# KTH-RPL/cloth-splatting

Hardware: AMD Instinct MI355X
Metric: rasterizer fwd+bwd rendered Mpix/s (scene_1, 800x800) (higher is better)
Workload: dtype f32

## Files before the change

### cloth-splatting_amd/csrc/csplat_k8_views_body.h

```cpp
    constexpr bool STAGE = true;
    if (tab.valid && *tab.valid == 0u) return;
    const int bx = (int)blockIdx.x + block0;
    const unsigned smask = tab.sharedmask;
    const bool put3 = !UNREAD && tab.unread == 0u;
#define PUTL(local, ptr, idx, val, bit)                                                    \
    do {                                                                                   \
        if (smask & (bit)) (local) += (val);                                               \
        else { float *p_ = (ptr) + (idx); *p_ = (accmask & (bit)) ? *p_ + (val) : (val); } \
    } while (0)
    static_assert(VL == 4 && K8_MAX_VIEWS <= 2 * VL, "one quad per Gaussian, at most two views per lane");
    constexpr int NG = NT / VL;
    __shared__ float s_in[STAGE ? NG * SH_ROW : 1];
    __shared__ float s_cam[CAM ? K8_MAX_VIEWS * NG * CAM_NC : 1];
    __shared__ float s_cpart[CAM ? CAM_PARTS * CAM_NC : 1];
    const int gi = threadIdx.x / VL, vl = threadIdx.x % VL;
    const int i = bx * NG + gi;
    const int rows = min(NG, P - bx * NG);
    if (STAGE) {
        stage_sh_rows<NT>(shs + (size_t)bx * NG * 48, rows, s_in);
        __syncthreads();
    }
    if (i < P) {
    float L_op = 0.f, L_col[3] = {0.f, 0.f, 0.f}, L_m3[3] = {0.f, 0.f, 0.f}, L_c6[6] = {0.f, 0.f, 0.f, 0.f, 0.f, 0.f};
    float L_sc[3] = {0.f, 0.f, 0.f}, L_rt[4] = {0.f, 0.f, 0.f, 0.f};
    bool vis_n = false;
    float a9_n[9];
    float dz_n = 0.f;
    auto load_record = [](const float *acc_, int i_, float (&a)[9], float &dz_) {
        const float4 *r4 = reinterpret_cast<const float4 *>(acc_ + (size_t)i_ * ACC_STRIDE);
        const float4 q0 = r4[0], q1 = r4[1], q2 = r4[2];
        a[0] = q0.x; a[1] = q0.y; a[2] = q0.z; a[3] = q0.w; a[4] = q1.x; a[5] = q1.y; a[6] = q1.z; a[7] = q1.w; a[8] = q2.x;
        if constexpr (DEPTH) dz_ = q2.y;
    };
    float e0[6] = {0.f, 0.f, 0.f, 0.f, 0.f, 0.f};
    if (vl < tab.n) {
        vis_n = tab.v[vl].radii[i] > 0;
        load_record(tab.v[vl].acc, i, a9_n, dz_n);
        if (vis_n && (tab.v[vl].accmask & CSPLAT_SCRATCH_ZEROED)) clear_record(tab.v[vl].acc, i);
    }
    for (int vi = vl; vi < tab.n; vi += VL) {
    const K8View &w = tab.v[vi];
    const Cam cam = w.cam;
    const Geom g = w.g;
    const int32_t *radii = w.radii;
    const float *acc = w.acc, *means3D = w.means3D, *rotations = w.rotations;
    float *dL_dmean2D = w.dL_dmean2D, *dL_dconic = w.dL_dconic, *dL_dopacity = w.dL_dopacity, *dL_dcolor = w.dL_dcolor;
    float *dL_dmean3D = w.dL_dmean3D, *dL_dcov3D = w.dL_dcov3D, *dL_dscale = w.dL_dscale, *dL_drot = w.dL_drot;
    const unsigned accmask = w.accmask;
    (void)radii; (void)acc;
    const bool vis = vis_n;
    float *const crow = s_cam + (CAM ? (vi * NG + gi) * CAM_NC : 0);
    float a9[9];
#pragma unroll
    for (int k = 0; k < 9; k++) a9[k] = vis ? a9_n[k] : 0.f;
    const float dz = vis ? dz_n : 0.f;
    moments_to_gradients(a9, vis ? g.conic_opacity[i] : make_float4(0.f, 0.f, 0.f, 0.f));
    a9[0] *= (float)cam.W; a9[1] *= (float)cam.H;
    if (vi + VL < tab.n) {
        const K8View &wn = tab.v[vi + VL];
        vis_n = wn.radii[i] > 0;
        load_record(wn.acc, i, a9_n, dz_n);
        if (vis_n && (wn.accmask & CSPLAT_SCRATCH_ZEROED)) clear_record(wn.acc, i);
    }
    dL_dmean2D[3 * i] = a9[0]; dL_dmean2D[3 * i + 1] = a9[1]; dL_dmean2D[3 * i + 2] = 0.f;
    if (put3) { dL_dconic[4 * i] = a9[2]; dL_dconic[4 * i + 1] = a9[3]; dL_dconic[4 * i + 2] = 0.f; dL_dconic[4 * i + 3] = a9[4]; }
    if constexpr (!AA) PUTL(L_op, dL_dopacity, i, a9[5], CSPLAT_ACC_OPACITY);
    if (put3) {
        PUTL(L_col[0], dL_dcolor, 3 * i, a9[6], CSPLAT_ACC_COLOR); PUTL(L_col[1], dL_dcolor, 3 * i + 1, a9[7], CSPLAT_ACC_COLOR);
        PUTL(L_col[2], dL_dcolor, 3 * i + 2, a9[8], CSPLAT_ACC_COLOR);
    }

// ... 3 lines not shown
    if (!vis) {
        if constexpr (AA) PUTL(L_op, dL_dopacity, i, 0.f, CSPLAT_ACC_OPACITY);
#pragma unroll
        for (int k = 0; k < 3; k++) PUTL(L_m3[k], dL_dmean3D, 3 * i + k, 0.f, CSPLAT_ACC_MEAN3D);
        if (put3)
#pragma unroll
            for (int k = 0; k < 6; k++) PUTL(L_c6[k], dL_dcov3D, 6 * i + k, 0.f, CSPLAT_ACC_COV3D);
        if (dL_dscale)
#pragma unroll
            for (int k = 0; k < 3; k++) PUTL(L_sc[k], dL_dscale, 3 * i + k, 0.f, CSPLAT_ACC_SCALE);
        if (dL_drot)
#pragma unroll
            for (int k = 0; k < 4; k++) PUTL(L_rt[k], dL_drot, 4 * i + k, 0.f, CSPLAT_ACC_ROT);
        if constexpr (CAM) cam_partials_zero(crow);
    } else {
    const float p[3] = {means3D[3 * i], means3D[3 * i + 1], means3D[3 * i + 2]};
    const float *view = cam.view, *proj = cam.proj;

    {
        float pv[3];
        view_point(p, view, pv);
        ProjJac pj;
        proj_jacobian(pv, cam, pj);
        float c6[6];
#pragma unroll
        for (int k = 0; k < 6; k++) c6[k] = g.cov3D[6 * i + k];
        float a, b, c;
        float aa_ga = 0.f, aa_gb = 0.f, aa_gc = 0.f;
        if constexpr (AA) {
            float a0, c0;
            cov2d_undilated(c6, pj, a0, b, c0);
            a = a0 + AA_DILATE; c = c0 + AA_DILATE;
            const float h = aa_backward(a0, b, c0, aa_opacities[i] * a9[5], aa_ga, aa_gb, aa_gc);
            PUTL(L_op, dL_dopacity, i, h * a9[5], CSPLAT_ACC_OPACITY);
        } else {
            cov2d_from_cov3d(c6, pj, a, b, c);
        }
        const float denom = a * c - b * b;
        const float denom2inv = 1.0f / ((denom * denom) + 0.0000001f);
        const float gcx = a9[2], gcy = a9[3], gcz = a9[4];
        float dL_da = 0.f, dL_db = 0.f, dL_dc = 0.f;
        const float *t0 = pj.t0, *t1 = pj.t1;
        if (denom2inv != 0.f) {
            dL_da = denom2inv * (-c * c * gcx + 2.f * b * c * gcy + (denom - a * c) * gcz);
            dL_dc = denom2inv * (-a * a * gcz + 2.f * a * b * gcy + (denom - a * c) * gcx);
            dL_db = denom2inv * 2.f * (b * c * gcx - (denom + 2.f * b * b) * gcy + a * b * gcz);
            if constexpr (AA) { dL_da += aa_ga; dL_db += aa_gb; dL_dc += aa_gc; }
            g6[0] = t0[0] * t0[0] * dL_da + t0[0] * t1[0] * dL_db + t1[0] * t1[0] * dL_dc;
// ... 30 lines not shown
            cam_partials_view(crow, p, dpv, cam.fx * tz, -(cam.fx * pj.tx) * tz2, cam.fy * tz, -(cam.fy * pj.ty) * tz2, dT0, dT1);
        }
    }
    {
        const float hw = proj[3] * p[0] + proj[7] * p[1] + proj[11] * p[2] + proj[15];
        const float m_w = 1.0f / (hw + 0.0000001f);
        const float mul1 = (proj[0] * p[0] + proj[4] * p[1] + proj[8] * p[2] + proj[12]) * m_w * m_w;
        const float mul2 = (proj[1] * p[0] + proj[5] * p[1] + proj[9] * p[2] + proj[13]) * m_w * m_w;
        const float gx2 = a9[0], gy2 = a9[1];
        dmean[0] += (proj[0] * m_w - proj[3] * mul1) * gx2 + (proj[1] * m_w - proj[3] * mul2) * gy2;
        dmean[1] += (proj[4] * m_w - proj[7] * mul1) * gx2 + (proj[5] * m_w - proj[7] * mul2) * gy2;
        dmean[2] += (proj[8] * m_w - proj[11] * mul1) * gx2 + (proj[9] * m_w - proj[11] * mul2) * gy2;
        if constexpr (CAM) cam_partials_proj(crow, p, gx2 * m_w, gy2 * m_w, -(mul1 * gx2 + mul2 * gy2));
    }
    if constexpr (CAM) { crow[32] = 0.f; crow[33] = 0.f; crow[34] = 0.f; }
    if (shs && dL_dsh) {
        const float *sh = (const float *)(s_in + gi * SH_ROW);
        const uint32_t cl = g.clamped[i];
        const float vx = p[0] - cam.campos[0], vy = p[1] - cam.campos[1], vz = p[2] - cam.campos[2];
        const float sum2 = vx * vx + vy * vy + vz * vz;
        const float len = sqrtf(sum2);
        const float x = vx / len, y = vy / len, z = vz / len;
        float ddx = 0.f, ddy = 0.f, ddz = 0.f;
        e[0] = x; e[1] = y; e[2] = z;
#pragma unroll
        for (int ch = 0; ch < 3; ch++) {
            const float dRGB = ((cl >> ch) & 1u) ? 0.f : a9[6 + ch];
            e[3 + ch] = dRGB;
            float dx_ = 0.f, dy_ = 0.f, dz_ = 0.f;
#define S(k) sh[(k) * 3 + ch]
            if (D > 0) {
                dx_ = -SH_C1 * S(3); dy_ = -SH_C1 * S(1); dz_ = SH_C1 * S(2);
                if (D > 1) {
// ... 22 lines not shown
        dmean[1] += (-vx * vy * ddx + (sum2 - vy * vy) * ddy - vz * vy * ddz) * invsum32;
        dmean[2] += (-vx * vz * ddx - vy * vz * ddy + (sum2 - vz * vz) * ddz) * invsum32;
        if constexpr (CAM) {
            const float dd = x * ddx + y * ddy + z * ddz, il = 1.f / len;
            crow[32] = (x * dd - ddx) * il; crow[33] = (y * dd - ddy) * il; crow[34] = (z * dd - ddz) * il;
        }
    }
    if constexpr (DEPTH) { dmean[0] += dz * view[2]; dmean[1] += dz * view[6]; dmean[2] += dz * view[10]; }
#pragma unroll
    for (int k = 0; k < 3; k++) PUTL(L_m3[k], dL_dmean3D, 3 * i + k, dmean[k], CSPLAT_ACC_MEAN3D);
    if (put3)
#pragma unroll
        for (int k = 0; k < 6; k++) PUTL(L_c6[k], dL_dcov3D, 6 * i + k, g6[k], CSPLAT_ACC_COV3D);

    if (!use_precomp_cov && dL_dscale && dL_drot) {
        const float q[4] = {rotations[4 * i], rotations[4 * i + 1], rotations[4 * i + 2], rotations[4 * i + 3]};
        float R[3][3];
        quat_to_rot(q, R);
        const float s[3] = {scale_mod * scales[3 * i], scale_mod * scales[3 * i + 1], scale_mod * scales[3 * i + 2]};
        const float dS[3][3] = {{g6[0], 0.5f * g6[1], 0.5f * g6[2]},
                                {0.5f * g6[1], g6[3], 0.5f * g6[4]},
                                {0.5f * g6[2], 0.5f * g6[4], g6[5]}};
        float dA[3][3];
#pragma unroll
        for (int r = 0; r < 3; r++)
#pragma unroll
            for (int k = 0; k < 3; k++)
                dA[r][k] = 2.f * (dS[r][0] * R[0][k] * s[k] + dS[r][1] * R[1][k] * s[k] + dS[r][2] * R[2][k] * s[k]);
#pragma unroll
        for (int k = 0; k < 3; k++) PUTL(L_sc[k], dL_dscale, 3 * i + k, dA[0][k] * R[0][k] + dA[1][k] * R[1][k] + dA[2][k] * R[2][k], CSPLAT_ACC_SCALE);
        float dR[3][3];
#pragma unroll
        for (int r = 0; r < 3; r++)
#pragma unroll
// ... 5 lines not shown
        const float dq2 = 2.f * (-2.f * qy * dR[0][0] + qx * dR[0][1] + qr * dR[0][2] + qx * dR[1][0] + qz * dR[1][2] -
                                    qr * dR[2][0] + qz * dR[2][1] - 2.f * qy * dR[2][2]);
        const float dq3 = 2.f * (-2.f * qz * dR[0][0] - qr * dR[0][1] + qx * dR[0][2] + qr * dR[1][0] - 2.f * qz * dR[1][1] +
                                    qy * dR[1][2] + qx * dR[2][0] + qy * dR[2][1]);
        PUTL(L_rt[0], dL_drot, 4 * i, dq0, CSPLAT_ACC_ROT); PUTL(L_rt[1], dL_drot, 4 * i + 1, dq1, CSPLAT_ACC_ROT);
        PUTL(L_rt[2], dL_drot, 4 * i + 2, dq2, CSPLAT_ACC_ROT); PUTL(L_rt[3], dL_drot, 4 * i + 3, dq3, CSPLAT_ACC_ROT);
    }
    }
    if (vi < VL) {
#pragma unroll
        for (int k = 0; k < 6; k++) e0[k] = e[k];
    } else {
#pragma unroll
        for (int k = 0; k < 6; k++) s_in[gi * SH_ROW + vl * 6 + k] = e[k];
    }
    }
    __builtin_amdgcn_wave_barrier();
    if (VL == 4) {
        auto quad_sum = [](float v) {
            v += __int_as_float(__builtin_amdgcn_update_dpp(0, __float_as_int(v), 0xB1, 0xF, 0xF, false));
            v += __int_as_float(__builtin_amdgcn_update_dpp(0, __float_as_int(v), 0x4E, 0xF, 0xF, false));
            return v;
        };
        L_op = quad_sum(L_op);
#pragma unroll
        for (int k = 0; k < 3; k++) { L_col[k] = quad_sum(L_col[k]); L_m3[k] = quad_sum(L_m3[k]); L_sc[k] = quad_sum(L_sc[k]); }
#pragma unroll
        for (int k = 0; k < 6; k++) L_c6[k] = quad_sum(L_c6[k]);
#pragma unroll
        for (int k = 0; k < 4; k++) L_rt[k] = quad_sum(L_rt[k]);
// ... 62 lines not shown
            for (int k = 0; k < 3; k++) PUTS(w.dL_dcolor, 3 * i + k, L_col[k], CSPLAT_ACC_COLOR);
#pragma unroll
        for (int k = 0; k < 3; k++) PUTS(w.dL_dmean3D, 3 * i + k, L_m3[k], CSPLAT_ACC_MEAN3D);
        if (put3)
#pragma unroll
            for (int k = 0; k < 6; k++) PUTS(w.dL_dcov3D, 6 * i + k, L_c6[k], CSPLAT_ACC_COV3D);
        if (w.dL_dscale)
#pragma unroll
            for (int k = 0; k < 3; k++) PUTS(w.dL_dscale, 3 * i + k, L_sc[k], CSPLAT_ACC_SCALE);
        if (w.dL_drot)
#pragma unroll
            for (int k = 0; k < 4; k++) PUTS(w.dL_drot, 4 * i + k, L_rt[k], CSPLAT_ACC_ROT);
#undef PUTS
    }
    }
    if constexpr (CAM)
        for (int vi = 0; vi < tab.n; vi++) cam_block_sum<NT>(s_cam + vi * NG * CAM_NC, rows, s_cpart, cam_slabs->p[vi] + (size_t)bx * CAM_NC);
#undef PUTL
```

### cloth-splatting_amd/csrc/csplat_raster.hip

```cpp
#include "csplat_common.h"

#include <atomic>
#include <cstring>
#include <chrono>
#include <mutex>
#include <type_traits>

#include "csplat_raster_math.h"
#include "csplat_raster_k1.h"
#include "csplat_raster_binning.h"
#include "csplat_raster_k5b_k6.h"

namespace {

constexpr int ACC_STRIDE = 16;

#define CSPLAT_ROWMASK_OP(OP, dst, src0, src1, RM)                                                                                  \
    asm("s_nop 1\n\tv_" OP "_f32_dpp %0, %1, %2 quad_perm:[0,1,2,3] row_mask:" RM " bank_mask:0xf" : "+v"(dst) : "v"(src0), "v"(src1))
__device__ __forceinline__ void rows_scan_mul(float f, float Tin, float &Tr, float &Tout) {
    const auto s16 = __builtin_amdgcn_permlane16_swap(__float_as_uint(f), __float_as_uint(f), false, false);
    const float ev = __uint_as_float(s16[0]), od = __uint_as_float(s16[1]);
    const float pr = ev * od;
    const auto s32 = __builtin_amdgcn_permlane32_swap(__float_as_uint(pr), __float_as_uint(pr), false, false);
    const float lo = __uint_as_float(s32[0]), hi = __uint_as_float(s32[1]);
// ... 597 lines not shown
        g_mail.tried = true;
        void *h = nullptr, *d = nullptr;
        if (hipHostMalloc(&h, MAIL_SLOTS * MAIL_WORDS * 4, hipHostMallocMapped | hipHostMallocPortable) == hipSuccess &&
            hipHostGetDevicePointer(&d, h, 0) == hipSuccess) {
            memset(h, 0, MAIL_SLOTS * MAIL_WORDS * 4);
            g_mail.host = (volatile uint32_t *)h;
            g_mail.dev = (uint32_t *)d;
        }
        (void)hipGetLastError();
    }
    return g_mail.host != nullptr;
}

unsigned long long *g_stamp_buf = nullptr;
size_t g_stamp_words = 0;

int tsort_mode(int P) { return (P < (1 << 24) ? 1 : 0) | (dbg(CSPLAT_DEBUG_SORT_RADIX_ONLY) ? 2 : 0) | (dbg(CSPLAT_DEBUG_SORT_RADIX_FALLBACK) ? 4 : 0); }

int higher_msb(uint32_t n) {
    int b = 0;
    while ((1u << b) < n && b < 31) b++;
    return b == 0 ? 1 : b;
}

hipEvent_t pooled_event() {
    constexpr int N = 256;
    static hipEvent_t ring[N];
    static std::atomic<unsigned> next{0};
    static std::mutex mu;
    const unsigned k = next.fetch_add(1) % N;
// ... 188 lines not shown
    for (int i = 0; i < V; i++) {
        const FwdTicket &t = g_tickets[tk[i]];
        K1View &k = tab.v[i];
        k.means3D = t.means3D; k.rotations = t.rotations; k.cam = t.cam; k.g = t.g; k.radii = t.radii; k.table = t.table;
        k.info = t.info; k.mailbox = t.mb_dev; k.ranges = t.ranges; k.tag = t.tag;
    }
    {
        ProfScope ps(PROF_K1, join);
        const bool stage = a.M == 16 && ((uintptr_t)a.shs & 15u) == 0;
        if (a.aa && stage)
            k_preprocess_views_aa<true><<<cdiv(P, K1V_G), 256, 0, join>>>(P, a.D, a.M, a.shs, a.opacities, a.scales, a.scale_modifier, tab,
                                                                        nocull_mode());
        else if (a.aa)
            k_preprocess_views_aa<false><<<cdiv(P, K1V_G), 256, 0, join>>>(P, a.D, a.M, a.shs, a.opacities, a.scales, a.scale_modifier, tab,
                                                                         nocull_mode());
        else if (stage)
            k_preprocess_views<true><<<cdiv(P, K1V_G), 256, 0, join>>>(P, a.D, a.M, a.shs, a.opacities, a.scales, a.scale_modifier, tab,
                                                                     nocull_mode());
        else
            k_preprocess_views<false><<<cdiv(P, K1V_G), 256, 0, join>>>(P, a.D, a.M, a.shs, a.opacities, a.scales, a.scale_modifier, tab,
                                                                      nocull_mode());
        LAUNCH_CHECK();
    }
    {
        ProfScope ps(PROF_K2, join);
        k_tile_count_views<<<dim3(nb, V), BUCKET_G, (size_t)tiles * 4, join>>>(P, tiles, tab);
        LAUNCH_CHECK();
        k_tile_colscan_views<<<dim3(cdiv(tiles, 256), V), 256, 0, join>>>(tiles, nb, tab);
        LAUNCH_CHECK();
        k_tile_scan_views<<<V, 1024, 0, join>>>(tiles, nb, tab);
// ... 849 lines not shown
    if (b_hi <= b_lo) return 0;
    auto go = [&](auto kernel, auto... extra) {
        kernel<<<b_hi - b_lo, 128, 0, join>>>(a.P, a.D, a.M, a.shs, a.scales, a.scale_modifier, 0, a.dL_dsh, tab, b_lo, extra...);
    };
    if (aa_of(a)) {
        if (depth && cam_k8) go(k_preprocess_bwd_views_aa<128, 4, true, true>, sl, a.opacities);
        else if (depth) go(k_preprocess_bwd_views_aa<128, 4, true, false>, sl, a.opacities);
        else if (cam_k8) go(k_preprocess_bwd_views_aa<128, 4, false, true>, sl, a.opacities);
        else go(k_preprocess_bwd_views_aa<128, 4, false, false>, sl, a.opacities);
    } else if (cam_k8) {
        if (depth) go(k_preprocess_bwd_views_cam<128, 4, true>, sl);
        else go(k_preprocess_bwd_views_cam<128, 4, false>, sl);
    } else if (depth) {
        go(k_preprocess_bwd_views_depth<128, 4>);
    } else {
        if (tab.unread) go(k_preprocess_bwd_views<128, 4, true>);
        else go(k_preprocess_bwd_views<128, 4, false>);
    }
    LAUNCH_CHECK();
    return 0;
}

struct GroupPlan {
    bool want_k7, want_k8, whole, shared, one_k8, det_mode, cam, cam_k8, feat;
    ScratchPath path;
    K8Table tab;
};
static void plan_group(int V, const csplat_view *v, unsigned parts, int nslices, GroupPlan &g) {
    g.want_k7 = (parts & 1u) != 0; g.want_k8 = (parts & 2u) != 0; g.whole = parts == 3u && nslices == 1;
    g.shared = false;
    for (int i = 0; i < V; i++) g.shared |= (v[i].accmask & ~(unsigned)(CSPLAT_SCRATCH_ZEROED | CSPLAT_K8_OUTPUTS_UNREAD)) != 0u;
// ... 287 lines not shown
```

### cloth-splatting_amd/csrc/csplat_raster_k1.h

```cpp
#pragma once

namespace {

template <bool STAGE, bool AA = false>
__device__ __forceinline__ void preprocess_body(int P, int D, int M, const float *__restrict__ means3D,
                                                const float *__restrict__ shs,
                                                const float *__restrict__ colors_precomp,
                                                const float *__restrict__ opacities,
                                                const float *__restrict__ scales, float scale_mod,
                                                const float *__restrict__ rotations,
                                                const float *__restrict__ cov3D_precomp, const Cam &cam, const Geom &g,
                                                int32_t *__restrict__ radii, int nocull, const float *s_shrows, int i, int srow) {
#pragma clang fp contract(off)
    if (i >= P) return;
    float depth = 0.f, px = 0.f, py = 0.f, cut = -1.f;
    float4 co = {0.f, 0.f, 0.f, 0.f};
    float rgb[3] = {0.f, 0.f, 0.f};
    float c6[6] = {0.f, 0.f, 0.f, 0.f, 0.f, 0.f};
    uint32_t clampbits = 0, touched = 0;
    int rad = 0;

    const float p[3] = {means3D[3 * i], means3D[3 * i + 1], means3D[3 * i + 2]};
    float pv[3];
    view_point(p, cam.view, pv);
    do {
        if (pv[2] <= NEAR_Z) break;
        const float *pr = cam.proj;
        const float hx = pr[0] * p[0] + pr[4] * p[1] + pr[8] * p[2] + pr[12];
        const float hy = pr[1] * p[0] + pr[5] * p[1] + pr[9] * p[2] + pr[13];
        const float hw = pr[3] * p[0] + pr[7] * p[1] + pr[11] * p[2] + pr[15];
        const float pw = 1.0f / (hw + 0.0000001f);
        const float ndcx = hx * pw, ndcy = hy * pw;
        if (cov3D_precomp) {
#pragma unroll
            for (int k = 0; k < 6; k++) c6[k] = cov3D_precomp[6 * i + k];
        } else {
            const float s[3] = {scales[3 * i], scales[3 * i + 1], scales[3 * i + 2]};
            const float q[4] = {rotations[4 * i], rotations[4 * i + 1], rotations[4 * i + 2], rotations[4 * i + 3]};
            cov3d_from_scale_rot(s, scale_mod, q, c6);
        }
        ProjJac pj;
        proj_jacobian(pv, cam, pj);
        float a, b, c;
        float aa_h = 1.f;
        if constexpr (AA) {
            float a0, c0;
            cov2d_undilated(c6, pj, a0, b, c0);
            a = a0 + AA_DILATE; c = c0 + AA_DILATE;
            aa_h = aa_factor(a0, b, c0);
        } else {
            cov2d_from_cov3d(c6, pj, a, b, c);
        }
        const float det = a * c - b * b;
// ... 34 lines not shown
                                  SH_C3[3] * z * (2.f * zz - 3.f * xx - 3.f * yy) * S(12) +
                                  SH_C3[4] * x * (4.f * zz - xx - yy) * S(13) + SH_C3[5] * z * (xx - yy) * S(14) +
                                  SH_C3[6] * x * (xx - 3.f * yy) * S(15);
                        }
                    }
                }
#undef S
                res += 0.5f;
                if (res < 0.f) clampbits |= (1u << ch);
                rgb[ch] = fmaxf(res, 0.f);
            }
        }
        depth = pv[2];
        rad = r;
        px = ix; py = iy;
        float op = opacities[i];
        if constexpr (AA) op = op * aa_h;
        co = make_float4(c * det_inv, -b * det_inv, a * det_inv, op);
        touched = (uint32_t)((maxy - miny) * (maxx - minx));
        const float cancel = 4e-7f * (a * c + b * b) / det;
        cut = cancel < 0.25f ? 2.f * lam1 * logf(255.f * op) * (1.0001f + 2.f * cancel) + 0.01f : 3.0e38f;
        if (nocull == 1) cut = 3.0e38f;
        if (nocull == 2) cut = cut * 4.f + 4.f;
    } while (0);

    g.depth[i] = depth;
    radii[i] = rad;
    g.xy[i] = make_float2(px, py);
    g.conic_opacity[i] = co;
#pragma unroll
    for (int k = 0; k < 3; k++) g.rgb[3 * i + k] = rgb[k];
#pragma unroll
    for (int k = 0; k < 6; k++) g.cov3D[6 * i + k] = c6[k];
    g.clamped[i] = clampbits;
    g.tiles_touched[i] = touched;
    g.cut2[i] = cut;
    g.pack[3 * (size_t)i] = make_float4(px, py, co.x, co.y);
    g.pack[3 * (size_t)i + 1] = make_float4(co.z, co.w, rgb[0], rgb[1]);
    g.pack[3 * (size_t)i + 2] = make_float4(rgb[2], depth, cut, 0.f);
}

template <bool STAGE>
__global__ __launch_bounds__(256) void k_preprocess(int P, int D, int M, const float *__restrict__ means3D,
                                                     const float *__restrict__ shs,
                                                     const float *__restrict__ colors_precomp,
                                                     const float *__restrict__ opacities,
                                                     const float *__restrict__ scales, float scale_mod,
                                                     const float *__restrict__ rotations,
                                                     const float *__restrict__ cov3D_precomp, Cam cam, Geom g,
                                                     int32_t *__restrict__ radii, int nocull) {
    __shared__ float s_shrows[STAGE ? 256 * SH_ROW : 1];
    if (STAGE) {
        const int base = blockIdx.x * 256;
        stage_sh_rows<256>(shs + (size_t)base * 48, min(256, P - base), s_shrows);
        __syncthreads();
    }
    preprocess_body<STAGE>(P, D, M, means3D, shs, colors_precomp, opacities, scales, scale_mod, rotations, cov3D_precomp, cam, g, radii,
                           nocull, s_shrows, (int)(blockIdx.x * blockDim.x + threadIdx.x), (int)threadIdx.x);
}
template <bool STAGE>
__global__ __launch_bounds__(256) void k_preprocess_aa(int P, int D, int M, const float *__restrict__ means3D,
                                                        const float *__restrict__ shs,
                                                        const float *__restrict__ colors_precomp,
                                                        const float *__restrict__ opacities,
                                                        const float *__restrict__ scales, float scale_mod,
                                                        const float *__restrict__ rotations,
                                                        const float *__restrict__ cov3D_precomp, Cam cam, Geom g,
                                                        int32_t *__restrict__ radii, int nocull) {
    __shared__ float s_shrows[STAGE ? 256 * SH_ROW : 1];
    if (STAGE) {
        const int base = blockIdx.x * 256;
        stage_sh_rows<256>(shs + (size_t)base * 48, min(256, P - base), s_shrows);
        __syncthreads();
    }
    preprocess_body<STAGE, true>(P, D, M, means3D, shs, colors_precomp, opacities, scales, scale_mod, rotations, cov3D_precomp, cam, g,
                                 radii, nocull, s_shrows, (int)(blockIdx.x * blockDim.x + threadIdx.x), (int)threadIdx.x);
}

struct K1View {
    const float *means3D, *rotations;
    Cam cam;
    Geom g;
    int32_t *radii;
    uint32_t *table, *info, *mailbox;
    int2 *ranges;
    uint32_t tag;
};
struct K1Table { int n; K1View v[RASTER_MAX_VIEWS]; };

constexpr int K1V_G = 64;
template <bool STAGE>
__global__ __launch_bounds__(256) void k_preprocess_views(int P, int D, int M, const float *__restrict__ shs,
                                                           const float *__restrict__ opacities,
                                                           const float *__restrict__ scales, float scale_mod, K1Table tab,
                                                           int nocull) {
    __shared__ float s_shrows[STAGE ? K1V_G * SH_ROW : 1];
    const int base = blockIdx.x * K1V_G;
    if (STAGE) {
        stage_sh_rows<256>(shs + (size_t)base * 48, min(K1V_G, P - base), s_shrows);
        __syncthreads();
    }
    const int lane = threadIdx.x & 63;
    for (int vi = threadIdx.x >> 6; vi < tab.n; vi += 4) {
        const K1View &w = tab.v[vi];
        preprocess_body<STAGE>(P, D, M, w.means3D, shs, nullptr, opacities, scales, scale_mod, w.rotations, nullptr, w.cam, w.g, w.radii, nocull,
                               s_shrows, base + lane, lane);
    }
}
template <bool STAGE>
__global__ __launch_bounds__(256) void k_preprocess_views_aa(int P, int D, int M, const float *__restrict__ shs,
                                                              const float *__restrict__ opacities,
                                                              const float *__restrict__ scales, float scale_mod, K1Table tab,
                                                              int nocull) {
    __shared__ float s_shrows[STAGE ? K1V_G * SH_ROW : 1];
    const int base = blockIdx.x * K1V_G;
    if (STAGE) {
        stage_sh_rows<256>(shs + (size_t)base * 48, min(K1V_G, P - base), s_shrows);
        __syncthreads();
    }
    const int lane = threadIdx.x & 63;
    for (int vi = threadIdx.x >> 6; vi < tab.n; vi += 4) {
        const K1View &w = tab.v[vi];
        preprocess_body<STAGE, true>(P, D, M, w.means3D, shs, nullptr, opacities, scales, scale_mod, w.rotations, nullptr, w.cam, w.g, w.radii,
                                     nocull, s_shrows, base + lane, lane);
    }
}

}
```

### cloth-splatting_amd/csrc/csplat_raster_k8.h

```cpp
#pragma once

namespace {

__device__ __forceinline__ void moments_to_gradients(float (&a9)[9], const float4 co) {
    const float h = -0.5f * co.w;
    const float mx = a9[0], my = a9[1];
    a9[0] = h * (co.x * mx + co.y * my);
    a9[1] = h * (co.z * my + co.y * mx);
    a9[2] *= h; a9[3] *= h; a9[4] *= h;
}
__device__ __forceinline__ void clear_record(const float *acc, int i) {
    float4 *p = reinterpret_cast<float4 *>(const_cast<float *>(acc) + (size_t)i * ACC_STRIDE);
    const float4 z = make_float4(0.f, 0.f, 0.f, 0.f);
    p[0] = z; p[1] = z; p[2] = z;
}
constexpr int CAM_NC = 35;
constexpr int CAM_PARTS = 8;
__device__ __forceinline__ void cam_partials_zero(float *row) {
#pragma unroll
    for (int k = 0; k < CAM_NC; k++) row[k] = 0.f;
}
__device__ __forceinline__ void cam_partials_view(float *row, const float p[3], const float dpv[3], float J00, float J02, float J11, float J12,
                                                  const float dT0[3], const float dT1[3]) {
#pragma unroll
// ... 315 lines not shown
    float *dL_dmean2D, *dL_dconic, *dL_dopacity, *dL_dcolor, *dL_dmean3D, *dL_dcov3D, *dL_dscale, *dL_drot;
    unsigned accmask;
};
struct K8Table {
    int n;
    unsigned sharedmask;
    unsigned unread;
    const uint32_t *valid;
    K8View v[RASTER_MAX_VIEWS];
};

struct CamSlabs {
    float *p[RASTER_MAX_VIEWS];
};
template <int NT, int VL, bool UNREAD>
__global__ __launch_bounds__(NT) void k_preprocess_bwd_views(int P, int D, int M, const float *__restrict__ shs,
                                                               const float *__restrict__ scales, float scale_mod,
                                                               int use_precomp_cov, float *__restrict__ dL_dsh, K8Table tab, int block0) {
    constexpr bool DEPTH = false, CAM = false, AA = false;
    const CamSlabs *const cam_slabs = nullptr;
    const float *const aa_opacities = nullptr;
    (void)aa_opacities;
#include "csplat_k8_views_body.h"
}
template <int NT, int VL>
__global__ __launch_bounds__(NT) void k_preprocess_bwd_views_depth(int P, int D, int M, const float *__restrict__ shs,
                                                                     const float *__restrict__ scales, float scale_mod,
                                                                     int use_precomp_cov, float *__restrict__ dL_dsh, K8Table tab, int block0) {
    constexpr bool DEPTH = true, CAM = false, AA = false, UNREAD = false;
    const CamSlabs *const cam_slabs = nullptr;
    const float *const aa_opacities = nullptr;
    (void)aa_opacities;
#include "csplat_k8_views_body.h"
}
template <int NT, int VL, bool DEPTH>
__global__ __launch_bounds__(NT) void k_preprocess_bwd_views_cam(int P, int D, int M, const float *__restrict__ shs,
                                                                   const float *__restrict__ scales, float scale_mod,
                                                                   int use_precomp_cov, float *__restrict__ dL_dsh, K8Table tab, int block0,
                                                                   CamSlabs slabs) {
    constexpr bool CAM = true, AA = false, UNREAD = false;
    const CamSlabs *const cam_slabs = &slabs;
    const float *const aa_opacities = nullptr;
    (void)aa_opacities;
#include "csplat_k8_views_body.h"
}
template <int NT, int VL, bool DEPTH, bool CAM>
__global__ __launch_bounds__(NT) void k_preprocess_bwd_views_aa(int P, int D, int M, const float *__restrict__ shs,
                                                                  const float *__restrict__ scales, float scale_mod,
                                                                  int use_precomp_cov, float *__restrict__ dL_dsh, K8Table tab, int block0,
                                                                  CamSlabs slabs, const float *__restrict__ opacities) {
    constexpr bool AA = true, UNREAD = false;
    const CamSlabs *const cam_slabs = &slabs;
    const float *const aa_opacities = opacities;
    (void)cam_slabs;
#include "csplat_k8_views_body.h"
}

constexpr int BG_BLOCKS = 256;
struct BgView {
    const float *final_T, *dL_dpix;
    float *slab;
    int npix;
};
struct BgTable {
    BgView v[RASTER_MAX_VIEWS];
};
// ... 65 lines not shown
```

Measured before the change: 4733.

## Hoist per-Gaussian input loads ahead of SH staging and prefetch next view

In the preprocess forward and backward view kernels, per-Gaussian inputs (means, cov3D, rotations, scales, conic/opacity, clamp bits) are now loaded into registers before the shared-memory SH staging barrier, and the next view's inputs are prefetched inside the per-view loop. SH staging is batched so all global loads are issued before the shared stores. Launch bounds gain occupancy hints, and optional timestamp-instrumented kernel variants are added. The aim is to hide global load latency behind the barrier, at the cost of more registers and possibly lower occupancy.

Measured after the change: 4788, median of 6. 1.01x the previous value.

```diff
diff --git a/cloth-splatting_amd/csrc/csplat_k8_views_body.h b/cloth-splatting_amd/csrc/csplat_k8_views_body.h
--- a/cloth-splatting_amd/csrc/csplat_k8_views_body.h
+++ b/cloth-splatting_amd/csrc/csplat_k8_views_body.h
@@ -16,11 +16,35 @@
     const int gi = threadIdx.x / VL, vl = threadIdx.x % VL;
     const int i = bx * NG + gi;
     const int rows = min(NG, P - bx * NG);
-    if (STAGE) {
-        stage_sh_rows<NT>(shs + (size_t)bx * NG * 48, rows, s_in);
-        __syncthreads();
-    }
-    if (i < P) {
+    if (tab.n <= 0) return;
+    auto mark = [&](int k, float dep) {
+        if constexpr (STAMP) StampMark{stamp_buf + (size_t)bx * 8}(k, dep);
+    };
+    mark(0, 0.f);
+    struct ViewIn {
+        float4 co;
+        float c6[6];
+        float p[3];
+        uint32_t cl;
+        float q[4];
+    };
+    const bool want_sh = shs && dL_dsh;
+    auto load_view_inputs = [&](const K8View &w_, int i_, ViewIn &o) {
+        const float4 *co_ = w_.g.conic_opacity;
+        const float *c6_ = w_.g.cov3D, *m3_ = w_.means3D, *rot_ = w_.rotations;
+        const uint32_t *cl_ = w_.g.clamped;
+        const bool rot_ok = !use_precomp_cov && rot_;
+        const float *rp_ = rot_ok ? rot_ : reinterpret_cast<const float *>(co_);
+        const int ri_ = rot_ok ? 4 * i_ : 0;
+        o.co = co_[i_];
+#pragma unroll
+        for (int k = 0; k < 6; k++) o.c6[k] = c6_[6 * i_ + k];
+#pragma unroll
+        for (int k = 0; k < 3; k++) o.p[k] = m3_[3 * i_ + k];
+        o.cl = cl_[i_];
+#pragma unroll
+        for (int k = 0; k < 4; k++) o.q[k] = rp_[ri_ + k];
+    };
     float L_op = 0.f, L_col[3] = {0.f, 0.f, 0.f}, L_m3[3] = {0.f, 0.f, 0.f}, L_c6[6] = {0.f, 0.f, 0.f, 0.f, 0.f, 0.f};
     float L_sc[3] = {0.f, 0.f, 0.f}, L_rt[4] = {0.f, 0.f, 0.f, 0.f};
     bool vis_n = false;
@@ -33,17 +57,39 @@
         if constexpr (DEPTH) dz_ = q2.y;
     };
     float e0[6] = {0.f, 0.f, 0.f, 0.f, 0.f, 0.f};
-    if (vl < tab.n) {
-        vis_n = tab.v[vl].radii[i] > 0;
-        load_record(tab.v[vl].acc, i, a9_n, dz_n);
-        if (vis_n && (tab.v[vl].accmask & CSPLAT_SCRATCH_ZEROED)) clear_record(tab.v[vl].acc, i);
-    }
+    ViewIn in;
+    const int il = min(i, P - 1);
+    const int v0 = min(vl, tab.n - 1);
+    const int32_t *radii0 = tab.v[v0].radii;
+    const float *acc0 = tab.v[v0].acc;
+    const unsigned accmask0 = tab.v[v0].accmask;
+    load_view_inputs(tab.v[v0], il, in);
+    vis_n = radii0[il] > 0;
+    load_record(acc0, il, a9_n, dz_n);
+    float sc3[3];
+    {
+        const bool sc_ok = !use_precomp_cov && scales;
+        const float *sp = sc_ok ? scales : reinterpret_cast<const float *>(tab.v[v0].g.conic_opacity);
+        const int si = sc_ok ? 3 * il : 0;
+#pragma unroll
+        for (int k = 0; k < 3; k++) sc3[k] = sp[si + k];
+    }
+    float aa_o = 0.f;
+    if constexpr (AA) aa_o = aa_opacities[il];
+    (void)aa_o;
+    if (STAGE) {
+        stage_sh_rows_batched<NT, NG>(shs + (size_t)bx * NG * 48, rows, s_in);
+        __syncthreads();
+    }
+    mark(1, 0.f);
+    if (i < P) {
+    vis_n = vis_n && vl < tab.n;
+    if (vis_n && (accmask0 & CSPLAT_SCRATCH_ZEROED)) clear_record(acc0, i);
     for (int vi = vl; vi < tab.n; vi += VL) {
     const K8View &w = tab.v[vi];
     const Cam cam = w.cam;
-    const Geom g = w.g;
     const int32_t *radii = w.radii;
-    const float *acc = w.acc, *means3D = w.means3D, *rotations = w.rotations;
+    const float *acc = w.acc;
     float *dL_dmean2D = w.dL_dmean2D, *dL_dconic = w.dL_dconic, *dL_dopacity = w.dL_dopacity, *dL_dcolor = w.dL_dcolor;
     float *dL_dmean3D = w.dL_dmean3D, *dL_dcov3D = w.dL_dcov3D, *dL_dscale = w.dL_dscale, *dL_drot = w.dL_drot;
     const unsigned accmask = w.accmask;
@@ -54,7 +100,9 @@
 #pragma unroll
     for (int k = 0; k < 9; k++) a9[k] = vis ? a9_n[k] : 0.f;
     const float dz = vis ? dz_n : 0.f;
-    moments_to_gradients(a9, vis ? g.conic_opacity[i] : make_float4(0.f, 0.f, 0.f, 0.f));
+    mark(2, a9_n[8]);
+    mark(3, in.co.w);
+    moments_to_gradients(a9, vis ? in.co : make_float4(0.f, 0.f, 0.f, 0.f));
     a9[0] *= (float)cam.W; a9[1] *= (float)cam.H;
     if (vi + VL < tab.n) {
         const K8View &wn = tab.v[vi + VL];
@@ -88,7 +136,7 @@
             for (int k = 0; k < 4; k++) PUTL(L_rt[k], dL_drot, 4 * i + k, 0.f, CSPLAT_ACC_ROT);
         if constexpr (CAM) cam_partials_zero(crow);
     } else {
-    const float p[3] = {means3D[3 * i], means3D[3 * i + 1], means3D[3 * i + 2]};
+    const float p[3] = {in.p[0], in.p[1], in.p[2]};
     const float *view = cam.view, *proj = cam.proj;
 
     {
@@ -98,14 +146,14 @@
         proj_jacobian(pv, cam, pj);
         float c6[6];
 #pragma unroll
-        for (int k = 0; k < 6; k++) c6[k] = g.cov3D[6 * i + k];
+        for (int k = 0; k < 6; k++) c6[k] = in.c6[k];
         float a, b, c;
         float aa_ga = 0.f, aa_gb = 0.f, aa_gc = 0.f;
         if constexpr (AA) {
             float a0, c0;
             cov2d_undilated(c6, pj, a0, b, c0);
             a = a0 + AA_DILATE; c = c0 + AA_DILATE;
-            const float h = aa_backward(a0, b, c0, aa_opacities[i] * a9[5], aa_ga, aa_gb, aa_gc);
+            const float h = aa_backward(a0, b, c0, aa_o * a9[5], aa_ga, aa_gb, aa_gc);
             PUTL(L_op, dL_dopacity, i, h * a9[5], CSPLAT_ACC_OPACITY);
         } else {
             cov2d_from_cov3d(c6, pj, a, b, c);
@@ -166,9 +214,9 @@
         if constexpr (CAM) cam_partials_proj(crow, p, gx2 * m_w, gy2 * m_w, -(mul1 * gx2 + mul2 * gy2));
     }
     if constexpr (CAM) { crow[32] = 0.f; crow[33] = 0.f; crow[34] = 0.f; }
-    if (shs && dL_dsh) {
+    if (want_sh) {
         const float *sh = (const float *)(s_in + gi * SH_ROW);
-        const uint32_t cl = g.clamped[i];
+        const uint32_t cl = in.cl;
         const float vx = p[0] - cam.campos[0], vy = p[1] - cam.campos[1], vz = p[2] - cam.campos[2];
         const float sum2 = vx * vx + vy * vy + vz * vz;
         const float len = sqrtf(sum2);
@@ -221,10 +269,11 @@
         for (int k = 0; k < 6; k++) PUTL(L_c6[k], dL_dcov3D, 6 * i + k, g6[k], CSPLAT_ACC_COV3D);
 
     if (!use_precomp_cov && dL_dscale && dL_drot) {
-        const float q[4] = {rotations[4 * i], rotations[4 * i + 1], rotations[4 * i + 2], rotations[4 * i + 3]};
+        const float q[4] = {in.q[0], in.q[1], in.q[2], in.q[3]};
         float R[3][3];
         quat_to_rot(q, R);
-        const float s[3] = {scale_mod * scales[3 * i], scale_mod * scales[3 * i + 1], scale_mod * scales[3 * i + 2]};
+        const float s[3] = {scale_mod * sc3[0], scale_mod * sc3[1], scale_mod * sc3[2]};
+        mark(4, s[2]);
         const float dS[3][3] = {{g6[0], 0.5f * g6[1], 0.5f * g6[2]},
                                 {0.5f * g6[1], g6[3], 0.5f * g6[4]},
                                 {0.5f * g6[2], 0.5f * g6[4], g6[5]}};
@@ -260,6 +309,7 @@
 #pragma unroll
         for (int k = 0; k < 6; k++) s_in[gi * SH_ROW + vl * 6 + k] = e[k];
     }
+    if (vi + VL < tab.n) load_view_inputs(tab.v[vi + VL], i, in);
     }
     __builtin_amdgcn_wave_barrier();
     if (VL == 4) {
@@ -352,6 +402,7 @@
 #undef PUTS
     }
     }
+    mark(5, 0.f);
     if constexpr (CAM)
         for (int vi = 0; vi < tab.n; vi++) cam_block_sum<NT>(s_cam + vi * NG * CAM_NC, rows, s_cpart, cam_slabs->p[vi] + (size_t)bx * CAM_NC);
 #undef PUTL
diff --git a/cloth-splatting_amd/csrc/csplat_raster.hip b/cloth-splatting_amd/csrc/csplat_raster.hip
--- a/cloth-splatting_amd/csrc/csplat_raster.hip
+++ b/cloth-splatting_amd/csrc/csplat_raster.hip
@@ -635,6 +635,9 @@
 
 unsigned long long *g_stamp_buf = nullptr;
 size_t g_stamp_words = 0;
+unsigned long long *per_gaussian_stamps(int P) {
+    return (g_stamp_buf && g_stamp_words == 8u * ((size_t)cdiv(P, 64) + (size_t)cdiv(P, 32))) ? g_stamp_buf : nullptr;
+}
 
 int tsort_mode(int P) { return (P < (1 << 24) ? 1 : 0) | (dbg(CSPLAT_DEBUG_SORT_RADIX_ONLY) ? 2 : 0) | (dbg(CSPLAT_DEBUG_SORT_RADIX_FALLBACK) ? 4 : 0); }
 
@@ -853,6 +856,9 @@
         else if (a.aa)
             k_preprocess_views_aa<false><<<cdiv(P, K1V_G), 256, 0, join>>>(P, a.D, a.M, a.shs, a.opacities, a.scales, a.scale_modifier, tab,
                                                                          nocull_mode());
+        else if (stage && per_gaussian_stamps(P))
+            k_preprocess_views_stamps<<<cdiv(P, K1V_G), 256, 0, join>>>(P, a.D, a.M, a.shs, a.opacities, a.scales, a.scale_modifier, tab,
+                                                                      nocull_mode(), per_gaussian_stamps(P));
         else if (stage)
             k_preprocess_views<true><<<cdiv(P, K1V_G), 256, 0, join>>>(P, a.D, a.M, a.shs, a.opacities, a.scales, a.scale_modifier, tab,
                                                                      nocull_mode());
@@ -1732,7 +1738,8 @@
     } else if (depth) {
         go(k_preprocess_bwd_views_depth<128, 4>);
     } else {
-        if (tab.unread) go(k_preprocess_bwd_views<128, 4, true>);
+        if (tab.unread && per_gaussian_stamps(a.P)) go(k_preprocess_bwd_views_stamps<128, 4>, per_gaussian_stamps(a.P) + (size_t)cdiv(a.P, 64) * 8);
+        else if (tab.unread) go(k_preprocess_bwd_views<128, 4, true>);
         else go(k_preprocess_bwd_views<128, 4, false>);
     }
     LAUNCH_CHECK();
diff --git a/cloth-splatting_amd/csrc/csplat_raster_k1.h b/cloth-splatting_amd/csrc/csplat_raster_k1.h
--- a/cloth-splatting_amd/csrc/csplat_raster_k1.h
+++ b/cloth-splatting_amd/csrc/csplat_raster_k1.h
@@ -2,15 +2,68 @@
 
 namespace {
 
-template <bool STAGE, bool AA = false>
-__device__ __forceinline__ void preprocess_body(int P, int D, int M, const float *__restrict__ means3D,
-                                                const float *__restrict__ shs,
-                                                const float *__restrict__ colors_precomp,
-                                                const float *__restrict__ opacities,
-                                                const float *__restrict__ scales, float scale_mod,
-                                                const float *__restrict__ rotations,
-                                                const float *__restrict__ cov3D_precomp, const Cam &cam, const Geom &g,
-                                                int32_t *__restrict__ radii, int nocull, const float *s_shrows, int i, int srow) {
+struct K1In {
+    float p[3];
+    float sq[7];
+    float op;
+};
+__device__ __forceinline__ void k1_request(int P, const float *__restrict__ means3D, const float *__restrict__ opacities,
+                                           const float *__restrict__ scales, const float *__restrict__ rotations,
+                                           const float *__restrict__ cov3D_precomp, int i, K1In &in) {
+    const int il = min(i, P - 1);
+#pragma unroll
+    for (int k = 0; k < 3; k++) in.p[k] = means3D[3 * il + k];
+    if (cov3D_precomp) {
+#pragma unroll
+        for (int k = 0; k < 6; k++) in.sq[k] = cov3D_precomp[6 * il + k];
+        in.sq[6] = 0.f;
+    } else {
+#pragma unroll
+        for (int k = 0; k < 3; k++) in.sq[k] = scales[3 * il + k];
+#pragma unroll
+        for (int k = 0; k < 4; k++) in.sq[3 + k] = rotations[4 * il + k];
+    }
+    in.op = opacities[il];
+}
+
+template <int NT, int ROWS>
+__device__ __forceinline__ void stage_sh_rows_batched(const float *__restrict__ src, int rows, float *s_rows) {
+    constexpr int N = (ROWS * 12 + NT - 1) / NT;
+    const float4 *src4 = reinterpret_cast<const float4 *>(src);
+    const int n = rows * 12;
+    float4 v[N];
+#pragma unroll
+    for (int k = 0; k < N; k++) v[k] = src4[min((int)threadIdx.x + k * NT, n - 1)];
+#pragma unroll
+    for (int k = 0; k < N; k++) {
+        const int t = (int)threadIdx.x + k * NT;
+        if (t < n) {
+            const int row = t / 12, c = (t - row * 12) * 4;
+            float *d = s_rows + row * SH_ROW + c;
+            d[0] = v[k].x; d[1] = v[k].y; d[2] = v[k].z; d[3] = v[k].w;
+        }
+    }
+}
+
+struct NoMark {
+    __device__ __forceinline__ void operator()(int, float) const {}
+};
+struct StampMark {
+    unsigned long long *at;
+    __device__ __forceinline__ void operator()(int k, float dep) const {
+        if (threadIdx.x == 0) {
+            asm volatile("" ::"v"(dep) : "memory");
+            at[k] = (unsigned long long)__builtin_amdgcn_s_memtime();
+            asm volatile("" ::: "memory");
+        }
+    }
+};
+
+template <bool STAGE, bool AA = false, class MK = NoMark>
+__device__ __forceinline__ void preprocess_body(int P, int D, int M, const K1In &in, const float *__restrict__ shs,
+                                                const float *__restrict__ colors_precomp, float scale_mod, bool cov_precomp,
+                                                const Cam &cam, const Geom &g, int32_t *__restrict__ radii, int nocull,
+                                                const float *s_shrows, int i, int srow, const MK &mark = MK()) {
 #pragma clang fp contract(off)
     if (i >= P) return;
     float depth = 0.f, px = 0.f, py = 0.f, cut = -1.f;
@@ -20,7 +73,8 @@
     uint32_t clampbits = 0, touched = 0;
     int rad = 0;
 
-    const float p[3] = {means3D[3 * i], means3D[3 * i + 1], means3D[3 * i + 2]};
+    const float p[3] = {in.p[0], in.p[1], in.p[2]};
+    mark(2, p[2]);
     float pv[3];
     view_point(p, cam.view, pv);
     do {
@@ -31,12 +85,13 @@
         const float hw = pr[3] * p[0] + pr[7] * p[1] + pr[11] * p[2] + pr[15];
         const float pw = 1.0f / (hw + 0.0000001f);
         const float ndcx = hx * pw, ndcy = hy * pw;
-        if (cov3D_precomp) {
-#pragma unroll
-            for (int k = 0; k < 6; k++) c6[k] = cov3D_precomp[6 * i + k];
+        if (cov_precomp) {
+#pragma unroll
+            for (int k = 0; k < 6; k++) c6[k] = in.sq[k];
         } else {
-            const float s[3] = {scales[3 * i], scales[3 * i + 1], scales[3 * i + 2]};
-            const float q[4] = {rotations[4 * i], rotations[4 * i + 1], rotations[4 * i + 2], rotations[4 * i + 3]};
+            const float s[3] = {in.sq[0], in.sq[1], in.sq[2]};
+            const float q[4] = {in.sq[3], in.sq[4], in.sq[5], in.sq[6]};
+            mark(3, q[3]);
             cov3d_from_scale_rot(s, scale_mod, q, c6);
         }
         ProjJac pj;
@@ -101,7 +156,8 @@
         depth = pv[2];
         rad = r;
         px = ix; py = iy;
-        float op = opacities[i];
+        float op = in.op;
+        mark(4, op);
         if constexpr (AA) op = op * aa_h;
         co = make_float4(c * det_inv, -b * det_inv, a * det_inv, op);
         touched = (uint32_t)((maxy - miny) * (maxx - minx));
@@ -125,6 +181,7 @@
     g.pack[3 * (size_t)i] = make_float4(px, py, co.x, co.y);
     g.pack[3 * (size_t)i + 1] = make_float4(co.z, co.w, rgb[0], rgb[1]);
     g.pack[3 * (size_t)i + 2] = make_float4(rgb[2], depth, cut, 0.f);
+    mark(5, 0.f);
 }
 
 template <bool STAGE>
@@ -137,13 +194,16 @@
                                                      const float *__restrict__ cov3D_precomp, Cam cam, Geom g,
                                                      int32_t *__restrict__ radii, int nocull) {
     __shared__ float s_shrows[STAGE ? 256 * SH_ROW : 1];
+    const int i = (int)(blockIdx.x * blockDim.x + threadIdx.x);
+    K1In in;
+    k1_request(P, means3D, opacities, scales, rotations, cov3D_precomp, i, in);
     if (STAGE) {
         const int base = blockIdx.x * 256;
         stage_sh_rows<256>(shs + (size_t)base * 48, min(256, P - base), s_shrows);
         __syncthreads();
     }
-    preprocess_body<STAGE>(P, D, M, means3D, shs, colors_precomp, opacities, scales, scale_mod, rotations, cov3D_precomp, cam, g, radii,
-                           nocull, s_shrows, (int)(blockIdx.x * blockDim.x + threadIdx.x), (int)threadIdx.x);
+    preprocess_body<STAGE>(P, D, M, in, shs, colors_precomp, scale_mod, cov3D_precomp != nullptr, cam, g, radii, nocull, s_shrows, i,
+                           (int)threadIdx.x);
 }
 template <bool STAGE>
 __global__ __launch_bounds__(256) void k_preprocess_aa(int P, int D, int M, const float *__restrict__ means3D,
@@ -155,13 +215,16 @@
                                                         const float *__restrict__ cov3D_precomp, Cam cam, Geom g,
                                                         int32_t *__restrict__ radii, int nocull) {
     __shared__ float s_shrows[STAGE ? 256 * SH_ROW : 1];
+    const int i = (int)(blockIdx.x * blockDim.x + threadIdx.x);
+    K1In in;
+    k1_request(P, means3D, opacities, scales, rotations, cov3D_precomp, i, in);
     if (STAGE) {
         const int base = blockIdx.x * 256;
         stage_sh_rows<256>(shs + (size_t)base * 48, min(256, P - base), s_shrows);
         __syncthreads();
     }
-    preprocess_body<STAGE, true>(P, D, M, means3D, shs, colors_precomp, opacities, scales, scale_mod, rotations, cov3D_precomp, cam, g,
-                                 radii, nocull, s_shrows, (int)(blockIdx.x * blockDim.x + threadIdx.x), (int)threadIdx.x);
+    preprocess_body<STAGE, true>(P, D, M, in, shs, colors_precomp, scale_mod, cov3D_precomp != nullptr, cam, g, radii, nocull, s_shrows, i,
+                                 (int)threadIdx.x);
 }
 
 struct K1View {
@@ -176,23 +239,38 @@
 struct K1Table { int n; K1View v[RASTER_MAX_VIEWS]; };
 
 constexpr int K1V_G = 64;
+template <bool STAGE, bool AA, class MK>
+__device__ __forceinline__ void preprocess_views(int P, int D, int M, const float *__restrict__ shs, const float *__restrict__ opacities,
+                                                 const float *__restrict__ scales, float scale_mod, const K1Table &tab, int nocull,
+                                                 float *s_shrows, const MK &mark) {
+    mark(0, 0.f);
+    const int base = blockIdx.x * K1V_G;
+    const int lane = threadIdx.x & 63;
+    if (tab.n <= 0) return;
+    const int wave = __builtin_amdgcn_readfirstlane((int)(threadIdx.x >> 6));
+    K1In in;
+    {
+        const K1View &w0 = tab.v[min(wave, tab.n - 1)];
+        k1_request(P, w0.means3D, opacities, scales, w0.rotations, nullptr, base + lane, in);
+    }
+    if (STAGE) {
+        stage_sh_rows_batched<256, K1V_G>(shs + (size_t)base * 48, min(K1V_G, P - base), s_shrows);
+        __syncthreads();
+    }
+    mark(1, 0.f);
+    for (int vi = wave; vi < tab.n; vi += 4) {
+        const K1View &w = tab.v[vi];
+        preprocess_body<STAGE, AA>(P, D, M, in, shs, nullptr, scale_mod, false, w.cam, w.g, w.radii, nocull, s_shrows, base + lane, lane, mark);
+        if (vi + 4 < tab.n) k1_request(P, tab.v[vi + 4].means3D, opacities, scales, tab.v[vi + 4].rotations, nullptr, base + lane, in);
+    }
+}
 template <bool STAGE>
 __global__ __launch_bounds__(256) void k_preprocess_views(int P, int D, int M, const float *__restrict__ shs,
                                                            const float *__restrict__ opacities,
                                                            const float *__restrict__ scales, float scale_mod, K1Table tab,
                                                            int nocull) {
     __shared__ float s_shrows[STAGE ? K1V_G * SH_ROW : 1];
-    const int base = blockIdx.x * K1V_G;
-    if (STAGE) {
-        stage_sh_rows<256>(shs + (size_t)base * 48, min(K1V_G, P - base), s_shrows);
-        __syncthreads();
-    }
-    const int lane = threadIdx.x & 63;
-    for (int vi = threadIdx.x >> 6; vi < tab.n; vi += 4) {
-        const K1View &w = tab.v[vi];
-        preprocess_body<STAGE>(P, D, M, w.means3D, shs, nullptr, opacities, scales, scale_mod, w.rotations, nullptr, w.cam, w.g, w.radii, nocull,
-                               s_shrows, base + lane, lane);
-    }
+    preprocess_views<STAGE, false>(P, D, M, shs, opacities, scales, scale_mod, tab, nocull, s_shrows, NoMark());
 }
 template <bool STAGE>
 __global__ __launch_bounds__(256) void k_preprocess_views_aa(int P, int D, int M, const float *__restrict__ shs,
@@ -200,17 +278,14 @@
                                                               const float *__restrict__ scales, float scale_mod, K1Table tab,
                                                               int nocull) {
     __shared__ float s_shrows[STAGE ? K1V_G * SH_ROW : 1];
-    const int base = blockIdx.x * K1V_G;
-    if (STAGE) {
-        stage_sh_rows<256>(shs + (size_t)base * 48, min(K1V_G, P - base), s_shrows);
-        __syncthreads();
-    }
-    const int lane = threadIdx.x & 63;
-    for (int vi = threadIdx.x >> 6; vi < tab.n; vi += 4) {
-        const K1View &w = tab.v[vi];
-        preprocess_body<STAGE, true>(P, D, M, w.means3D, shs, nullptr, opacities, scales, scale_mod, w.rotations, nullptr, w.cam, w.g, w.radii,
-                                     nocull, s_shrows, base + lane, lane);
-    }
-}
-
-}
+    preprocess_views<STAGE, true>(P, D, M, shs, opacities, scales, scale_mod, tab, nocull, s_shrows, NoMark());
+}
+__global__ __launch_bounds__(256) void k_preprocess_views_stamps(int P, int D, int M, const float *__restrict__ shs,
+                                                                  const float *__restrict__ opacities,
+                                                                  const float *__restrict__ scales, float scale_mod, K1Table tab,
+                                                                  int nocull, unsigned long long *stamp_buf) {
+    __shared__ float s_shrows[K1V_G * SH_ROW];
+    preprocess_views<true, false>(P, D, M, shs, opacities, scales, scale_mod, tab, nocull, s_shrows, StampMark{stamp_buf + (size_t)blockIdx.x * 8});
+}
+
+}
diff --git a/cloth-splatting_amd/csrc/csplat_raster_k8.h b/cloth-splatting_amd/csrc/csplat_raster_k8.h
--- a/cloth-splatting_amd/csrc/csplat_raster_k8.h
+++ b/cloth-splatting_amd/csrc/csplat_raster_k8.h
@@ -353,20 +353,35 @@
     float *p[RASTER_MAX_VIEWS];
 };
 template <int NT, int VL, bool UNREAD>
-__global__ __launch_bounds__(NT) void k_preprocess_bwd_views(int P, int D, int M, const float *__restrict__ shs,
+__global__ __launch_bounds__(NT, UNREAD ? 4 : 3) void k_preprocess_bwd_views(int P, int D, int M, const float *__restrict__ shs,
                                                                const float *__restrict__ scales, float scale_mod,
                                                                int use_precomp_cov, float *__restrict__ dL_dsh, K8Table tab, int block0) {
-    constexpr bool DEPTH = false, CAM = false, AA = false;
+    constexpr bool DEPTH = false, CAM = false, AA = false, STAMP = false;
+    unsigned long long *const stamp_buf = nullptr;
+    (void)stamp_buf;
     const CamSlabs *const cam_slabs = nullptr;
     const float *const aa_opacities = nullptr;
     (void)aa_opacities;
 #include "csplat_k8_views_body.h"
 }
 template <int NT, int VL>
+__global__ __launch_bounds__(NT, 4) void k_preprocess_bwd_views_stamps(int P, int D, int M, const float *__restrict__ shs,
+                                                                        const float *__restrict__ scales, float scale_mod,
+                                                                        int use_precomp_cov, float *__restrict__ dL_dsh, K8Table tab, int block0,
+                                                                        unsigned long long *stamp_buf) {
+    constexpr bool DEPTH = false, CAM = false, AA = false, UNREAD = true, STAMP = true;
+    const CamSlabs *const cam_slabs = nullptr;
+    const float *const aa_opacities = nullptr;
+    (void)aa_opacities;
+#include "csplat_k8_views_body.h"
+}
+template <int NT, int VL>
 __global__ __launch_bounds__(NT) void k_preprocess_bwd_views_depth(int P, int D, int M, const float *__restrict__ shs,
                                                                      const float *__restrict__ scales, float scale_mod,
                                                                      int use_precomp_cov, float *__restrict__ dL_dsh, K8Table tab, int block0) {
-    constexpr bool DEPTH = true, CAM = false, AA = false, UNREAD = false;
+    constexpr bool DEPTH = true, CAM = false, AA = false, UNREAD = false, STAMP = false;
+    unsigned long long *const stamp_buf = nullptr;
+    (void)stamp_buf;
     const CamSlabs *const cam_slabs = nullptr;
     const float *const aa_opacities = nullptr;
     (void)aa_opacities;
@@ -377,7 +392,9 @@
                                                                    const float *__restrict__ scales, float scale_mod,
                                                                    int use_precomp_cov, float *__restrict__ dL_dsh, K8Table tab, int block0,
                                                                    CamSlabs slabs) {
-    constexpr bool CAM = true, AA = false, UNREAD = false;
+    constexpr bool CAM = true, AA = false, UNREAD = false, STAMP = false;
+    unsigned long long *const stamp_buf = nullptr;
+    (void)stamp_buf;
     const CamSlabs *const cam_slabs = &slabs;
     const float *const aa_opacities = nullptr;
     (void)aa_opacities;
@@ -388,7 +405,9 @@
                                                                   const float *__restrict__ scales, float scale_mod,
                                                                   int use_precomp_cov, float *__restrict__ dL_dsh, K8Table tab, int block0,
                                                                   CamSlabs slabs, const float *__restrict__ opacities) {
-    constexpr bool AA = true, UNREAD = false;
+    constexpr bool AA = true, UNREAD = false, STAMP = false;
+    unsigned long long *const stamp_buf = nullptr;
+    (void)stamp_buf;
     const CamSlabs *const cam_slabs = &slabs;
     const float *const aa_opacities = opacities;
     (void)cam_slabs;
```
